# JokerJohn/Cloud_Map_Evaluation

Hardware: AMD Instinct MI355X
Metric: Mpts/sec full metric suite (CD+MME+AWD) on 50M-pt pair (higher is better)
Workload: dtype f64

## Files before the change

### cloud_map_evaluation_amd/csrc/me_internal.hpp

```cpp
#pragma once

#include <hip/hip_runtime.h>

#include <algorithm>
#include <cstdint>
#include <cstdlib>
#include <cstdio>
#include <map>
#include <string>
#include <vector>

#include "../../include/mapeval_hip.h"

namespace me {

constexpr int kFan = 8;
constexpr int kMaxLevels = 17;
constexpr int kMortonBits = 21;

struct DevBuf {
    void *p = nullptr;
    size_t bytes = 0;
    bool owned = true;
    ~DevBuf() { release(); }
// ... 773 lines not shown
    unsigned int lo = (unsigned int) __double2loint(v), hi = (unsigned int) __double2hiint(v);
    auto a = __builtin_amdgcn_permlane16_swap(lo, lo, false, false);
    auto b = __builtin_amdgcn_permlane16_swap(hi, hi, false, false);
    v = __hiloint2double((int) b[0], (int) a[0]) + __hiloint2double((int) b[1], (int) a[1]);
    lo = (unsigned int) __double2loint(v);
    hi = (unsigned int) __double2hiint(v);
    auto c = __builtin_amdgcn_permlane32_swap(lo, lo, false, false);
    auto d = __builtin_amdgcn_permlane32_swap(hi, hi, false, false);
    return __hiloint2double((int) d[0], (int) c[0]) + __hiloint2double((int) d[1], (int) c[1]);
}
template <int STAGE>
__device__ __forceinline__ int octet_partner_i(int v) {
    constexpr int ctrl = STAGE == 0 ? 0xB1 : (STAGE == 1 ? 0x4E : 0x141);
    return __builtin_amdgcn_update_dpp(0, v, ctrl, 0xF, 0xF, true);
}
template <int STAGE>
__device__ __forceinline__ double octet_partner_d(double v) {
    return __hiloint2double(octet_partner_i<STAGE>(__double2hiint(v)), octet_partner_i<STAGE>(__double2loint(v)));
}
template <int STAGE>
__device__ __forceinline__ long long octet_partner_ll(long long v) {
    const unsigned int lo = (unsigned int) octet_partner_i<STAGE>((int) (unsigned int) v);
    const unsigned int hi = (unsigned int) octet_partner_i<STAGE>((int) (unsigned int) ((unsigned long long) v >> 32));
    return (long long) (((unsigned long long) hi << 32) | lo);
}
__device__ __forceinline__ int wave_min_i(int v) {
    v = min(v, __builtin_amdgcn_update_dpp(0, v, 0xB1, 0xF, 0xF, true));
    v = min(v, __builtin_amdgcn_update_dpp(0, v, 0x4E, 0xF, 0xF, true));
    v = min(v, __builtin_amdgcn_update_dpp(0, v, 0x141, 0xF, 0xF, true));
    v = min(v, __builtin_amdgcn_update_dpp(0, v, 0x140, 0xF, 0xF, true));
    return min(min(__builtin_amdgcn_readlane(v, 0), __builtin_amdgcn_readlane(v, 16)),
               min(__builtin_amdgcn_readlane(v, 32), __builtin_amdgcn_readlane(v, 48)));
}
__device__ __forceinline__ int wave_max_i(int v) {
    v = max(v, __builtin_amdgcn_update_dpp(0, v, 0xB1, 0xF, 0xF, true));
    v = max(v, __builtin_amdgcn_update_dpp(0, v, 0x4E, 0xF, 0xF, true));
    v = max(v, __builtin_amdgcn_update_dpp(0, v, 0x141, 0xF, 0xF, true));
    v = max(v, __builtin_amdgcn_update_dpp(0, v, 0x140, 0xF, 0xF, true));
    return max(max(__builtin_amdgcn_readlane(v, 0), __builtin_amdgcn_readlane(v, 16)),
               max(__builtin_amdgcn_readlane(v, 32), __builtin_amdgcn_readlane(v, 48)));
}

constexpr int kGroupR = 2;
constexpr int kGroupTab = 343;
constexpr int kGroupTab2 = (2 * kGroupR + 5) * (2 * kGroupR + 5) * (2 * kGroupR + 5);

__host__ __device__ constexpr unsigned int recip14(int n) {
    return (unsigned int) (((n < 4 ? 0x1556200040000000ULL : 0x09250AAB0CCD1000ULL) >> (16 * (n & 3))) & 0xffffULL);
}
constexpr bool recip14_exact() {
    for (int n = 1; n <= 7; ++n)
        for (unsigned int t = 0; t < 5461; ++t)
            if (((t * recip14(n)) >> 14) != t / (unsigned int) n) return false;
    return true;
}
static_assert(recip14_exact(), "t / n as (t * recip14(n)) >> 14");
__host__ __device__ constexpr unsigned int spread11_32(unsigned int x) {
    x = (x | x << 16) & 0x070000ffu;
    x = (x | x << 8) & 0x0700f00fu;
    x = (x | x << 4) & 0x430c30c3u;
    x = (x | x << 2) & 0x49249249u;
    return x;
}
__host__ __device__ constexpr unsigned long long spread21_halves(unsigned int x) {
    return (unsigned long long) spread11_32(x & 0x3ffu) | ((unsigned long long) spread11_32((x >> 10) & 0x7ffu) << 30);
}
constexpr unsigned long long spread21_ladder(unsigned long long x) {
    x &= 0x1fffffULL;
    x = (x | x << 32) & 0x1f00000000ffffULL;
    x = (x | x << 16) & 0x1f0000ff0000ffULL;
    x = (x | x << 8) & 0x100f00f00f00f00fULL;
    x = (x | x << 4) & 0x10c30c30c30c30c3ULL;
    x = (x | x << 2) & 0x1249249249249249ULL;
    return x;
}
constexpr bool spread21_halves_exact() {
    for (unsigned int i = 0; i < 21; ++i) {
        const unsigned int a = 1u << i, b = (2u << i) - 1u, c = 0x1fffffu & ~(a - 1u);
        if (spread21_halves(a) != spread21_ladder(a) || spread21_halves(b) != spread21_ladder(b) || spread21_halves(c) != spread21_ladder(c)) return false;
    }
    for (unsigned int x = 0; x < 0x200000u; x += 4099u)
        if (spread21_halves(x) != spread21_ladder(x)) return false;
    return true;
}
static_assert(spread21_halves_exact(), "spread21 from 32-bit halves");
constexpr int kGroupRowsEnt = 240;
template <int H = 1, bool CULL = false, int R = kGroupR, bool MLP = false, bool ENT = false>
__device__ __forceinline__ bool wave_group_table(bool pending, int cx, int cy, int cz, const GridView &g, int cell_lim,
                                                 int lane, int2 *tab, GroupBox &box, int *n_keys_out = nullptr,
                                                 unsigned int *rows = nullptr, unsigned short *tcell = nullptr,
                                                 unsigned int *tabc = nullptr, const unsigned int *cell_aux = nullptr,
                                                 int *leader_out = nullptr) {
    const unsigned long long pm = __ballot(pending);
#ifdef ME_LEADER_FIRST
    const int leader = __ffsll((long long) pm) - 1;
#else
    const int rank = __popcll(pm & ((1ULL << lane) - 1ULL));
    const int n_pending = __popcll(pm);
    int leader = __ffsll((long long) __ballot(pending && rank == (n_pending >> 1))) - 1;
#ifndef ME_LEADER_MIDDLE
    {
        auto group_size = [&](int l) {
            const int ax = readlane_i(cx, l), ay = readlane_i(cy, l), az = readlane_i(cz, l);
            const int ux = cx - ax, uy = cy - ay, uz = cz - az;
            return __popcll(__ballot(pending && ux >= -R && ux <= R && uy >= -R && uy <= R && uz >= -R && uz <= R));
        };
        int best = group_size(leader);
        if (best < n_pending && n_pending >= 8) {
#pragma unroll
            for (int c = 1; c <= 5; ++c) {
                if (c == 3) continue;
                const int l = __ffsll((long long) __ballot(pending && rank == ((c * n_pending) / 6))) - 1;
                const int b = group_size(l);
                if (b > best) {
                    best = b;
                    leader = l;
                }
            }
        }
    }
#endif
#endif
    if (leader_out) *leader_out = leader;
    const int lx = readlane_i(cx, leader), ly = readlane_i(cy, leader), lz = readlane_i(cz, leader);
    const int ex = cx - lx, ey = cy - ly, ez = cz - lz;
    const bool in = pending && ex >= -R && ex <= R && ey >= -R && ey <= R && ez >= -R && ez <= R;
    const int x0 = __builtin_amdgcn_readfirstlane(wave_min_i(in ? cx : lx)) - H;
    const int x1 = __builtin_amdgcn_readfirstlane(wave_max_i(in ? cx : lx)) + H;
    const int y0 = __builtin_amdgcn_readfirstlane(wave_min_i(in ? cy : ly)) - H;
    const int y1 = __builtin_amdgcn_readfirstlane(wave_max_i(in ? cy : ly)) + H;
    const int z0 = __builtin_amdgcn_readfirstlane(wave_min_i(in ? cz : lz)) - H;
    const int z1 = __builtin_amdgcn_readfirstlane(wave_max_i(in ? cz : lz)) + H;
    const int nx = x1 - x0 + 1, ny = y1 - y0 + 1, nz = z1 - z0 + 1;
    const int n_keys = nx * ny * nz;
    if (n_keys_out) *n_keys_out = n_keys;
    box.x0 = x0;
    box.y0 = y0;
    box.z0 = z0;
    box.nx = nx;
    box.ny = ny;
    static_assert(!ENT || (H == 1 && R <= 2 && CULL && !MLP), "ENT: the <= 7 x 7 x 7 box of the stream kernels, with the cull");
    const unsigned int mx = ENT ? recip14(nx) : 0u, my = ENT ? recip14(ny) : 0u;
    unsigned long long *ykey = ENT ? reinterpret_cast<unsigned long long *>(rows + 128) : nullptr, *xkey = ENT ? ykey + 49 : nullptr;
    if (CULL) {
        const int n_rows = ny * nz;
        if (lane < n_rows) rows[lane] = 0u;
        __builtin_amdgcn_fence(__ATOMIC_ACQ_REL, "wavefront");
        __builtin_amdgcn_wave_barrier();
        if (in) atomicOr(&rows[(cy - y0) + ny * (cz - z0)], 1u << (cx - x0));
        __builtin_amdgcn_fence(__ATOMIC_ACQ_REL, "wavefront");
        __builtin_amdgcn_wave_barrier();
        if (lane < n_rows) {
            const int rz = ENT ? (int) (((unsigned int) lane * my) >> 14) : lane / ny, ry = lane - rz * ny;
            unsigned int m = 0;
            for (int dz = -H; dz <= H; ++dz)
                for (int dy = -H; dy <= H; ++dy) {
                    const int yy = ry + dy, zz = rz + dz;
                    if (yy >= 0 && yy < ny && zz >= 0 && zz < nz) m |= rows[yy + ny * zz];
                }
            unsigned int d = m;
#pragma unroll
            for (int s = 1; s <= H; ++s) d |= (m << s) | (m >> s);
            if (ENT) {
                const int iy = y0 + ry, iz = z0 + rz;
                const unsigned int okx = ((1u << (cell_lim - x0 < nx ? cell_lim - x0 : nx)) - 1u) & ~((1u << (x0 < 0 ? -x0 : 0)) - 1u);
                d = (iy >= 0 && iy < cell_lim && iz >= 0 && iz < cell_lim) ? d & okx : 0u;
                ykey[lane] = (spread21_halves((unsigned int) iy & 0x1fffffu) << 1) | (spread21_halves((unsigned int) iz & 0x1fffffu) << 2);
            }
            rows[64 + lane] = d;
        }
        if (ENT && lane < nx) xkey[lane] = spread21_halves((unsigned int) (x0 + lane) & 0x1fffffu);
        __builtin_amdgcn_fence(__ATOMIC_ACQ_REL, "wavefront");
        __builtin_amdgcn_wave_barrier();
    }
    if (MLP) {
        constexpr int NIT = ((2 * R + 1 + 2 * H) * (2 * R + 1 + 2 * H) * (2 * R + 1 + 2 * H) + 63) / 64;
        unsigned long long key[NIT], got[NIT];
        unsigned int slot[NIT];
        bool want[NIT];
#pragma unroll
        for (int i = 0; i < NIT; ++i) {
            const int t = lane + 64 * i;
            const int tx = t % nx, ty = (t / nx) % ny, tz = t / (nx * ny);
            const int ix = x0 + tx, iy = y0 + ty, iz = z0 + tz;
            want[i] = t < n_keys && ix >= 0 && iy >= 0 && iz >= 0 && ix < cell_lim && iy < cell_lim && iz < cell_lim;
            if (CULL) want[i] = want[i] && ((rows[64 + (t < n_keys ? ty + ny * tz : 0)] >> tx) & 1u);
            key[i] = spread21((unsigned long long) ix) | (spread21((unsigned long long) iy) << 1) | (spread21((unsigned long long) iz) << 2);
            slot[i] = (unsigned int) hash_u64(key[i]) & g.hmask;
            got[i] = kEmptyKey;
            if (tcell && t < n_keys) tcell[t] = (unsigned short) (tx | (ty << 3) | (tz << 6));
        }
#pragma unroll
        for (int i = 0; i < NIT; ++i)
            if (want[i]) got[i] = g.hkeys[slot[i]];
        int ci[NIT];
#pragma unroll
        for (int i = 0; i < NIT; ++i) {
            while (want[i] && got[i] != key[i] && got[i] != kEmptyKey) {
                slot[i] = (slot[i] + 1) & g.hmask;
                got[i] = g.hkeys[slot[i]];
            }
            want[i] = want[i] && got[i] == key[i];
            ci[i] = 0;
        }
#pragma unroll
        for (int i = 0; i < NIT; ++i)
            if (want[i]) ci[i] = (int) g.hvals[slot[i]];
        unsigned int cs0[NIT], cs1[NIT], ax[NIT];
#pragma unroll
        for (int i = 0; i < NIT; ++i) {
            cs0[i] = cs1[i] = ax[i] = 0;
            if (want[i]) {
                cs0[i] = g.cell_start[ci[i]];
                cs1[i] = g.cell_start[ci[i] + 1];
                if (tabc) ax[i] = cell_aux[ci[i]];
            }
        }
#pragma unroll
        for (int i = 0; i < NIT; ++i) {
            const int t = lane + 64 * i;
            if (t < n_keys) {
                tab[t] = make_int2((int) cs0[i], (int) (cs1[i] - cs0[i]));
                if (tabc) tabc[t] = ax[i];
            }
        }
    } else if (ENT) {
        for (int t = lane; t < n_keys; t += 64) {
            const unsigned int q = ((unsigned int) t * mx) >> 14, tx = (unsigned int) t - q * (unsigned int) nx;
            int2 run = make_int2(0, 0);
            if ((rows[64 + q] >> tx) & 1u) {
                const unsigned long long key = ykey[q] | xkey[tx];
                unsigned int s = (unsigned int) hash_u64(key) & g.hmask;
                for (;;) {
                    uint4 e = *reinterpret_cast<const uint4 *>(g.hent + s);
                    asm volatile("" : "+v"(e.x), "+v"(e.y), "+v"(e.z), "+v"(e.w));
                    const unsigned long long k = ((unsigned long long) e.y << 32) | e.x;
                    if (k == key) {
                        run = make_int2((int) e.z, (int) e.w);
                        break;
                    }
                    if (k == kEmptyKey) break;
                    s = (s + 1) & g.hmask;
                }
            }
            tab[t] = run;
            if (tcell) {
                const unsigned int tz = (q * my) >> 14, ty = q - tz * (unsigned int) ny;
                tcell[t] = (unsigned short) (tx | (ty << 3) | (tz << 6));
            }
        }
    } else
    for (int t = lane; t < n_keys; t += 64) {
        const int tx = t % nx, ty = (t / nx) % ny, tz = t / (nx * ny);
        const int ix = x0 + tx, iy = y0 + ty, iz = z0 + tz;
        int2 run = make_int2(0, 0);
        unsigned int aux = 0;
        bool want = ix >= 0 && iy >= 0 && iz >= 0 && ix < cell_lim && iy < cell_lim && iz < cell_lim;
        if (CULL) want = want && ((rows[64 + ty + ny * tz] >> tx) & 1u);
        if (want) {
            const unsigned long long key = spread21((unsigned long long) ix) | (spread21((unsigned long long) iy) << 1) |
                                           (spread21((unsigned long long) iz) << 2);
            const int ci = hash_lookup(g.hkeys, g.hvals, g.hmask, key);
            if (ci >= 0) {
                run.x = (int) g.cell_start[ci];
                run.y = (int) g.cell_start[ci + 1] - run.x;
                if (tabc) aux = cell_aux[ci];
            }
        }
        tab[t] = run;
        if (tabc) tabc[t] = aux;
        if (tcell) tcell[t] = (unsigned short) (tx | (ty << 3) | (tz << 6));
    }
    __builtin_amdgcn_fence(__ATOMIC_ACQ_REL, "wavefront");
    __builtin_amdgcn_wave_barrier();
    return in;
}
constexpr int kGroupRows = 128;

template <bool MERGE = false, class F>
__device__ __forceinline__ void wave_for_each_run(const int2 *tab, int n_keys, int lane, F &&f) {
    for (int base = 0; base < n_keys; base += 64) {
        const int t = base + lane;
        const int cnt = (t < n_keys) ? tab[t].y : 0;
        unsigned long long m = __ballot(cnt > 0);
        while (m) {
            const int n = __ffsll((long long) m) - 1;
            m &= m - 1;
            const int2 run = tab[base + n];
            const int cs = __builtin_amdgcn_readfirstlane(run.x);
            int cc = __builtin_amdgcn_readfirstlane(run.y);
            if (MERGE) {
                while (m) {
                    const int n2 = __ffsll((long long) m) - 1;
                    const int2 nx = tab[base + n2];
                    if (__builtin_amdgcn_readfirstlane(nx.x) != cs + cc) break;
                    cc += __builtin_amdgcn_readfirstlane(nx.y);
                    m &= m - 1;
                }
            }
            f(cs, cs + cc, base + n);
        }
    }
}
#endif

}
```

### cloud_map_evaluation_amd/csrc/me_mme.hip

```cpp
#include <cmath>
#include <cstdlib>

#include "me_internal.hpp"

#ifndef ME_MME_DEPTH
#define ME_MME_DEPTH 2
#endif
#ifndef ME_MME_DBG
#define ME_MME_DBG 0
#endif

namespace me {

__device__ __forceinline__ double half2_sum_d(double v) {
    unsigned int lo = (unsigned int) __double2loint(v), hi = (unsigned int) __double2hiint(v);
    auto c = __builtin_amdgcn_permlane32_swap(lo, lo, false, false);
    auto d = __builtin_amdgcn_permlane32_swap(hi, hi, false, false);
    return __hiloint2double((int) d[0], (int) c[0]) + __hiloint2double((int) d[1], (int) c[1]);
}


#ifdef ME_MME_STATS
__device__ unsigned long long g_mme_stat[8];
#endif

struct alignas(16) MmeTileRec {
    float4 f;
    double2 xy;
    double z;
    double pad;
};
static_assert(sizeof(MmeTileRec) == 48, "tile record layout");
template <class T>
__device__ __forceinline__ T lds_load(unsigned int addr) {
#if defined(__HIP_DEVICE_COMPILE__)
    return *reinterpret_cast<const __attribute__((address_space(3))) T *>((size_t) addr);
#else
    (void) addr;
    return T{};
#endif
}

template <int TILE, int WAVES>
__global__ void __launch_bounds__(256) __attribute__((amdgpu_waves_per_eu(WAVES, WAVES)))
k_mme3(const SPoint *__restrict__ sp, const unsigned long long *__restrict__ codes, long long i_begin, long long i_end,
       GridView g, FrameView fr, SlabView slab, double r2, int min_k, double *__restrict__ ent_s,
       unsigned char *__restrict__ valid_s, double *__restrict__ part_sum, long long *__restrict__ part_cnt,
       unsigned int xcd_chunk, int dbg, double cell_h, float thr_lo, float thr_hi, unsigned long long *__restrict__ part_pairs,
       unsigned int *__restrict__ refine_list, unsigned int *__restrict__ refine_count, double cond) {
    static_assert(TILE * sizeof(MmeTileRec) >= kGroupRowsEnt * 4, "the row masks and keys of the round's table alias the tile");
    (void) fr;
    (void) cell_h;
    const unsigned int vb = xcd_virtual_block(blockIdx.x, gridDim.x, xcd_chunk);
    const unsigned int loc = vb * blockDim.x + threadIdx.x;
    bool active = i_begin + (long long) loc < i_end;
    const int shift3 = 3 * g.shift;
    const int cell_lim = 1 << (kMortonBits - g.shift);

    unsigned long long mycell = ~0ULL;
    if (active) {
        const long long i = i_begin + (long long) loc;
        mycell = codes[i] >> shift3;
        if (slab.axis >= 0) {
            const SPoint q = sp[i];
            if (!slab_owned(slab, q.x, q.y, q.z)) {
                ent_s[i] = 0.0;
                valid_s[i] = 0;
                active = false;
            }
        }
    }
    bool done = !active;

    __shared__ int2 s_tab[4][kGroupTab + 1];
    __shared__ MmeTileRec s_rec[4][TILE];
    const int wv = __builtin_amdgcn_readfirstlane((int) (threadIdx.x >> 6));
    int2 *tab = s_tab[wv];
    MmeTileRec *trec = s_rec[wv];
    const unsigned int trec_lds = (unsigned int) (size_t) trec;
    const int lane = threadIdx.x & 63;

    unsigned int wave_pairs = 0;
    double det_keep = 0.0;
    bool have_det = false;
    bool thin = false;
#ifdef ME_MME_STATS
    int st_round = 0;
#endif
    while (__ballot(!done)) {
        GroupBox bx;
        int nk = 0, leader = 0;
        const int cx = (int) compact21(mycell), cy = (int) compact21(mycell >> 1), cz = (int) compact21(mycell >> 2);
        const bool in = wave_group_table<1, true, kGroupR, false, true>(!done, cx, cy, cz, g, cell_lim, lane, tab, bx, &nk, reinterpret_cast<unsigned int *>(trec),
                                                  nullptr, nullptr, nullptr, &leader);
        double qx = 0, qy = 0, qz = 0;
        if (!done) {
            unsigned int loc_q = loc;
            asm volatile("" : "+v"(loc_q));
            const SPoint q = sp[i_begin + (long long) loc_q];
            qx = q.x;
            qy = q.y;
            qz = q.z;
        }
        const double ox = uniform_f64(__hiloint2double(__builtin_amdgcn_readlane(__double2hiint(qx), leader), __builtin_amdgcn_readlane(__double2loint(qx), leader)));
        const double oy = uniform_f64(__hiloint2double(__builtin_amdgcn_readlane(__double2hiint(qy), leader), __builtin_amdgcn_readlane(__double2loint(qy), leader)));
        const double oz = uniform_f64(__hiloint2double(__builtin_amdgcn_readlane(__double2hiint(qz), leader), __builtin_amdgcn_readlane(__double2loint(qz), leader)));
        const double rx = qx - ox, ry = qy - oy, rz = qz - oz;
        const float ax = (float) (-2.0 * rx), ay = (float) (-2.0 * ry), az = (float) (-2.0 * rz);
        const float s = fmaf(az, az, fmaf(ay, ay, ax * ax));
        const float t_hi = (in && dbg != 2) ? fmaf(-0.25f, s, thr_hi) : -INFINITY;
        const float t_lo = (in && dbg != 2) ? fmaf(-0.25f, s, thr_lo) : -INFINITY;
        int k = -1;
        double s1x = -rx, s1y = -ry, s1z = -rz;
        double sxx = -(rx * rx), sxy = -(rx * ry), sxz = -(rx * rz), syy = -(ry * ry), syz = -(ry * rz), szz = -(rz * rz);
        if (!in || dbg == 2) {
            k = 0;
            s1x = s1y = s1z = sxx = sxy = sxz = syy = syz = szz = 0.0;
        }
#ifdef ME_MME_STATS
        int st_cand = 0;
#endif
        auto test = [&](const float4 &c, unsigned int ra, int gj) {
            const float u = fmaf(c.x, ax, fmaf(c.y, ay, fmaf(c.z, az, c.w)));
            const bool hi = u < t_hi;
            const unsigned long long mh = __ballot(hi);
            if (mh) {
                bool acc = u < t_lo;
                if (__builtin_expect(mh != __ballot(acc), 0)) {
                    asm volatile("; band: exact test" ::: "memory");
                    unsigned int loc_b = loc;
                    asm volatile("" : "+v"(loc_b));
                    const SPoint qe = sp[i_begin + (long long) loc_b];
                    const SPoint pe = sp[gj];
                    const double ex = pe.x - qe.x, ey = pe.y - qe.y, ez = pe.z - qe.z;
                    const double d2 = (ex * ex + ey * ey) + ez * ez;
                    acc = acc || (hi && d2 < r2);
                }
                if (acc) {
                    const double2 pxy = lds_load<double2>(ra + 16);
                    const double dx = pxy.x, dy = pxy.y, dz = lds_load<double>(ra + 32);
                    ++k;
                    s1x += dx;
                    s1y += dy;
                    s1z += dz;
                    sxx = fma(dx, dx, sxx);
                    sxy = fma(dx, dy, sxy);
                    sxz = fma(dx, dz, sxz);
                    syy = fma(dy, dy, syy);
                    syz = fma(dy, dz, syz);
                    szz = fma(dz, dz, szz);
                }
            }
        };
        if (dbg != 1) wave_for_each_run(tab, nk, lane, [&](int cs, int ce, int) {
            for (int base = cs; base < ce; base += TILE) {
                const int n = min(TILE, ce - base);
#ifdef ME_MME_STATS
                st_cand += n;
#endif
                if (lane < n) {
                    const SPoint p = sp[base + lane];
                    const double px = p.x - ox, py = p.y - oy, pz = p.z - oz;
                    const float fx = (float) px, fy = (float) py, fz = (float) pz;
                    const double w = ((double) fx * (double) fx + (double) fy * (double) fy) + (double) fz * (double) fz;
                    trec[lane].f = make_float4(fx, fy, fz, (float) w);
                    trec[lane].xy = make_double2(px, py);
                    trec[lane].z = pz;
                }
                __builtin_amdgcn_fence(__ATOMIC_ACQ_REL, "wavefront");
                __builtin_amdgcn_wave_barrier();
                int j = (dbg == 3) ? n : 0;
                unsigned int ra = trec_lds;
                asm volatile("" : "+v"(ra));
                for (; j + 2 <= n; j += 2) {
                    const float4 c0 = lds_load<float4>(ra), c1 = lds_load<float4>(ra + (unsigned int) sizeof(MmeTileRec));
                    test(c0, ra, base + j);
                    test(c1, ra + (unsigned int) sizeof(MmeTileRec), base + j + 1);
                    ra += 2u * (unsigned int) sizeof(MmeTileRec);
                    asm volatile("" : "+v"(ra));
                }
                for (; j < n; ++j) {
                    const float4 c0 = lds_load<float4>(ra);
                    test(c0, ra, base + j);
                    ra += (unsigned int) sizeof(MmeTileRec);
                    asm volatile("" : "+v"(ra));
                }
                __builtin_amdgcn_fence(__ATOMIC_ACQ_REL, "wavefront");
                __builtin_amdgcn_wave_barrier();
            }
        });
#ifdef ME_MME_STATS
        {
            int ka = in ? k : 0;
            for (int o = 32; o > 0; o >>= 1) ka += __shfl_xor(ka, o, 64);
            const int served = __popcll(__ballot(in));
            if (lane == 0) {
                atomicAdd(&g_mme_stat[0], 1ULL);
                atomicAdd(&g_mme_stat[1], (unsigned long long) st_cand);
                atomicAdd(&g_mme_stat[2], (unsigned long long) served);
                atomicAdd(&g_mme_stat[3], (unsigned long long) ka);
                if (st_round > 0) {
                    atomicAdd(&g_mme_stat[4], 1ULL);
                    atomicAdd(&g_mme_stat[5], (unsigned long long) st_cand);
                    atomicAdd(&g_mme_stat[6], (unsigned long long) served);
                }
            }
            ++st_round;
        }
#endif
        if (part_pairs) {
            int ka = in ? k : 0;
            for (int o = 32; o > 0; o >>= 1) ka += __shfl_xor(ka, o, 64);
            wave_pairs += (unsigned int) __builtin_amdgcn_readfirstlane(ka);
        }
        if (in) {
            done = true;
            const int kk = k;
            if (kk >= min_k) {
                const double inv_k = 1.0 / (double) kk, inv_km1 = 1.0 / (double) (kk - 1);
                const double cxx = (sxx - s1x * s1x * inv_k) * inv_km1;
                const double cxy = (sxy - s1x * s1y * inv_k) * inv_km1;
                const double cxz = (sxz - s1x * s1z * inv_k) * inv_km1;
                const double cyy = (syy - s1y * s1y * inv_k) * inv_km1;
                const double cyz = (syz - s1y * s1z * inv_k) * inv_km1;
                const double czz = (szz - s1z * s1z * inv_k) * inv_km1;
                det_keep = cxx * (cyy * czz - cyz * cyz) - cxy * (cxy * czz - cyz * cxz) + cxz * (cxy * cyz - cyy * cxz);
                have_det = true;
                const double tr = (cxx + cyy) + czz;
                thin = det_keep < 0.25 * tr * tr * cond;
            }
        }
        __builtin_amdgcn_wave_barrier();
    }
    if (refine_list) {
        const unsigned long long tm = __ballot(thin);
        if (tm) {
            unsigned int base = 0;
            if (lane == 0) base = atomicAdd(refine_count, (unsigned int) __popcll(tm));
            base = (unsigned int) readlane_i((int) base, 0);
            if (thin) refine_list[base + (unsigned int) __popcll(tm & ((1ULL << lane) - 1ULL))] = loc;
        }
    }
    double H = 0.0;
    bool ok = false;
    if (active) {
        if (have_det) {
            const double h = 0.5 * log(2.0 * M_PI * M_E * det_keep);
            if (!isnan(h) && !isinf(h)) {
                H = h;
                ok = true;
            }
        }
        unsigned int loc_e = loc;
        asm volatile("" : "+v"(loc_e));
        const long long i = i_begin + (long long) loc_e;
        ent_s[i] = H;
        valid_s[i] = ok ? 1 : 0;
    }
    __shared__ double smd[4];
    __shared__ long long smi[4];
    const double bs = block_sum_256(H, smd);
    const long long bc = block_sum_256_ll(ok ? 1LL : 0LL, smi);
    if (threadIdx.x == 0) {
        part_sum[blockIdx.x] = bs;
        part_cnt[blockIdx.x] = bc;
    }
    if (part_pairs) {
        __shared__ unsigned int smp[4];
        if (lane == 0) smp[wv] = wave_pairs;
        __syncthreads();
        if (threadIdx.x == 0) part_pairs[blockIdx.x] = (unsigned long long) smp[0] + smp[1] + smp[2] + smp[3];
    }
}


constexpr int kRefineBlock = 256;
__global__ void __launch_bounds__(kRefineBlock)
k_mme_refine(const SPoint *__restrict__ sp, const unsigned long long *__restrict__ codes, long long i_begin, GridView g, double r2,
             int min_k, const unsigned int *__restrict__ list, unsigned int n_list, double *__restrict__ ent_s,
             unsigned char *__restrict__ valid_s) {
    __shared__ int2 s_runs[kRefineBlock / 8][28];
    const int sub = threadIdx.x & 7, oct = threadIdx.x >> 3;
    const unsigned int t = blockIdx.x * (kRefineBlock / 8) + oct;
    const bool alive = t < n_list;
    const long long i = i_begin + (long long) (alive ? list[t] : 0u);
    const SPoint q = sp[alive ? i : i_begin];
    const unsigned long long cell = codes[alive ? i : i_begin] >> (3 * g.shift);
    const int cx = (int) compact21(cell), cy = (int) compact21(cell >> 1), cz = (int) compact21(cell >> 2);
    const int cell_lim = 1 << (kMortonBits - g.shift);
    {
        unsigned long long key[4], got[4];
        unsigned int slot[4];
        bool want[4];
#pragma unroll
        for (int u = 0; u < 4; ++u) {
            const int c = sub + 8 * u;
            const int ix = cx + (c % 3) - 1, iy = cy + ((c / 3) % 3) - 1, iz = cz + (c / 9) - 1;
            want[u] = alive && c < 27 && ix >= 0 && iy >= 0 && iz >= 0 && ix < cell_lim && iy < cell_lim && iz < cell_lim;
            key[u] = spread21((unsigned long long) ix) | (spread21((unsigned long long) iy) << 1) | (spread21((unsigned long long) iz) << 2);
            slot[u] = (unsigned int) hash_u64(key[u]) & g.hmask;
            got[u] = kEmptyKey;
        }
#pragma unroll
        for (int u = 0; u < 4; ++u)
            if (want[u]) got[u] = g.hkeys[slot[u]];
        unsigned int ci[4], c0[4], c1[4];
#pragma unroll
        for (int u = 0; u < 4; ++u) {
            while (want[u] && got[u] != key[u] && got[u] != kEmptyKey) {
                slot[u] = (slot[u] + 1) & g.hmask;
                got[u] = g.hkeys[slot[u]];
            }
            want[u] = want[u] && got[u] == key[u];
            ci[u] = 0;
        }
#pragma unroll
        for (int u = 0; u < 4; ++u)
            if (want[u]) ci[u] = g.hvals[slot[u]];
#pragma unroll
        for (int u = 0; u < 4; ++u) {
            c0[u] = c1[u] = 0;
            if (want[u]) {
                c0[u] = g.cell_start[ci[u]];
                c1[u] = g.cell_start[ci[u] + 1];
            }
        }
#pragma unroll
        for (int u = 0; u < 4; ++u)
            if (sub + 8 * u < 27) s_runs[oct][sub + 8 * u] = make_int2((int) c0[u], (int) (c1[u] - c0[u]));
    }
    __builtin_amdgcn_fence(__ATOMIC_ACQ_REL, "wavefront");
    __builtin_amdgcn_wave_barrier();
    auto scan = [&](auto &&f) {
        for (int c = 0; c < 27; ++c) {
            const int2 run = s_runs[oct][c];
            for (int j0 = 0; j0 < run.y; j0 += 32) {
                SPoint p[4];
#pragma unroll
                for (int u = 0; u < 4; ++u) p[u] = sp[run.x + min(j0 + sub + 8 * u, run.y - 1)];
#pragma unroll
                for (int u = 0; u < 4; ++u) {
                    const double dx = p[u].x - q.x, dy = p[u].y - q.y, dz = p[u].z - q.z;
                    const double d2 = (dx * dx + dy * dy) + dz * dz;
                    if (j0 + sub + 8 * u < run.y && d2 < r2) f(dx, dy, dz);
                }
            }
        }
    };
    auto oct_sum = [](double v) {
        v += octet_partner_d<0>(v);
        v += octet_partner_d<1>(v);
        v += octet_partner_d<2>(v);
        return v;
    };
    int cnt = 0;
    double s1x = 0, s1y = 0, s1z = 0;
    scan([&](double dx, double dy, double dz) {
        ++cnt;
        s1x += dx;
        s1y += dy;
        s1z += dz;
    });
    cnt += octet_partner_i<0>(cnt);
    cnt += octet_partner_i<1>(cnt);
    cnt += octet_partner_i<2>(cnt);
    s1x = oct_sum(s1x);
    s1y = oct_sum(s1y);
    s1z = oct_sum(s1z);
    const int kk = cnt - 1;
    double H = 0.0;
    bool ok = false;
    if (kk >= min_k) {
        const double mx = s1x / (double) kk, my = s1y / (double) kk, mz = s1z / (double) kk;
        double sxx = 0, sxy = 0, sxz = 0, syy = 0, syz = 0, szz = 0;
        scan([&](double dx, double dy, double dz) {
            const double ex = dx - mx, ey = dy - my, ez = dz - mz;
            sxx = fma(ex, ex, sxx);
            sxy = fma(ex, ey, sxy);
            sxz = fma(ex, ez, sxz);
            syy = fma(ey, ey, syy);
            syz = fma(ey, ez, syz);
            szz = fma(ez, ez, szz);
        });
        sxx = oct_sum(sxx);
        sxy = oct_sum(sxy);
        sxz = oct_sum(sxz);
        syy = oct_sum(syy);
        syz = oct_sum(syz);
        szz = oct_sum(szz);
        sxx -= mx * mx;
        sxy -= mx * my;
        sxz -= mx * mz;
        syy -= my * my;
        syz -= my * mz;
        szz -= mz * mz;
        const double inv = 1.0 / (double) (kk - 1);
        const double cxx = sxx * inv, cxy = sxy * inv, cxz = sxz * inv, cyy = syy * inv, cyz = syz * inv, czz = szz * inv;
        const double det = cxx * (cyy * czz - cyz * cyz) - cxy * (cxy * czz - cyz * cxz) + cxz * (cxy * cyz - cyy * cxz);
        const double h = 0.5 * log(2.0 * M_PI * M_E * det);
        if (!isnan(h) && !isinf(h)) {
            H = h;
            ok = true;
        }
    }
    if (alive && sub == 0) {
        ent_s[i] = H;
        valid_s[i] = ok ? 1 : 0;
    }
}

__global__ void __launch_bounds__(256)
k_mme_resum(const double *__restrict__ ent_s, const unsigned char *__restrict__ valid_s, long long i_begin, long long i_end,
            double *__restrict__ part_sum, long long *__restrict__ part_cnt) {
    const long long i = i_begin + (long long) blockIdx.x * 256 + threadIdx.x;
    double H = 0.0;
    long long ok = 0;
    if (i < i_end) {
        H = ent_s[i];
        ok = valid_s[i] ? 1 : 0;
    }
    __shared__ double smd[4];
    __shared__ long long smi[4];
    const double bs = block_sum_256(H, smd);
    const long long bc = block_sum_256_ll(ok, smi);
    if (threadIdx.x == 0) {
        part_sum[blockIdx.x] = bs;
        part_cnt[blockIdx.x] = bc;
    }
}

__global__ void __launch_bounds__(256) k_sum_u64(const unsigned long long *__restrict__ v, long long n, unsigned long long *__restrict__ out) {
    long long s = 0;
    for (long long i = threadIdx.x; i < n; i += 256) s += (long long) v[i];
    __shared__ long long sm[4];
    const long long r = block_sum_256_ll(s, sm);
    if (threadIdx.x == 0) *out += (unsigned long long) r;
}

#ifdef ME_AB
#include "me_mme_kernels_ab.inc"
#endif

__global__ void k_mme_unpermute(const SPoint *__restrict__ sp, long long i_begin, long long i_end,
                                const double *__restrict__ ent_s, const unsigned char *__restrict__ valid_s,
                                double *__restrict__ ent_o, unsigned char *__restrict__ valid_o) {
    const long long i = i_begin + (long long) blockIdx.x * blockDim.x + threadIdx.x;
    if (i >= i_end) return;
    const long long o = sp[i].idx;
    if (ent_o) ent_o[o] = ent_s[i];
    if (valid_o) valid_o[o] = valid_s[i];
}

__global__ void __launch_bounds__(256)
k_mme_final(const double *__restrict__ ps, const long long *__restrict__ pc, long long nb, long long chunk,
            double *__restrict__ out_s, long long *__restrict__ out_c) {
    double s = 0;
    long long c = 0;
    const long long b0 = (long long) blockIdx.x * chunk, b1 = b0 + chunk < nb ? b0 + chunk : nb;
    for (long long b = b0 + threadIdx.x; b < b1; b += 256) {
        s += ps[b];
        c += pc[b];
    }
    __shared__ double smd[4];
    __shared__ long long smi[4];
    const double rs = block_sum_256(s, smd);
    const long long rc = block_sum_256_ll(c, smi);
    if (threadIdx.x == 0) {
        out_s[blockIdx.x] = rs;
        out_c[blockIdx.x] = rc;
    }
}

static int mme_unpermute_to_host(me_ctx *ctx, Cloud &c, long long b, long long e, double *entropies, uint8_t *valid) {
    const long long n = c.n;
    DevBuf &eo = ctx->tmp[2], &vo = ctx->tmp[3];
    ME_CHECK(ctx, eo.ensure((size_t) n * 8));
    ME_CHECK(ctx, vo.ensure((size_t) n));
    if (ctx->shard_world > 1) {
        ME_CHECK(ctx, hipMemsetAsync(eo.p, 0, (size_t) n * 8, ctx->stream));
        ME_CHECK(ctx, hipMemsetAsync(vo.p, 0, (size_t) n, ctx->stream));
    }
    if (e > b)
        hipLaunchKernelGGL(k_mme_unpermute, dim3((unsigned int) ((e - b + 255) / 256)), dim3(256), 0, ctx->stream, c.sp.as<SPoint>(), b, e,
                           c.mme_ent.as<double>(), c.mme_val.as<unsigned char>(), entropies ? eo.as<double>() : nullptr,
                           valid ? vo.as<unsigned char>() : nullptr);
    if (entropies) ME_TRY(copy_d2h(ctx, entropies, eo.p, (size_t) n * 8));
    if (valid) ME_TRY(copy_d2h(ctx, valid, vo.p, (size_t) n));
    return ME_OK;
}

__global__ void k_mme_repermute(const SPoint *__restrict__ sp, long long n, const double *__restrict__ ent_o,
                                const unsigned char *__restrict__ valid_o, double *__restrict__ ent_s, unsigned char *__restrict__ valid_s) {
    const long long i = (long long) blockIdx.x * blockDim.x + threadIdx.x;
    if (i >= n) return;
    const long long o = sp[i].idx;
    ent_s[i] = ent_o[o];
    valid_s[i] = valid_o[o];
}

int mme_carry_out(me_ctx *ctx, int slot) {
    Cloud &c = ctx->cloud[slot];
    if (!c.mme_have || c.n == 0) return ME_OK;
    ME_CHECK(ctx, ctx->mme_keep_e.ensure((size_t) c.n * 8));
    ME_CHECK(ctx, ctx->mme_keep_v.ensure((size_t) c.n));
    hipLaunchKernelGGL(k_mme_unpermute, dim3((unsigned int) ((c.n + 255) / 256)), dim3(256), 0, ctx->stream, c.sp.as<SPoint>(), 0LL, c.n,
                       c.mme_ent.as<double>(), c.mme_val.as<unsigned char>(), ctx->mme_keep_e.as<double>(),
                       ctx->mme_keep_v.as<unsigned char>());
    ctx->mme_keep_n = c.n;
    return ME_OK;
}

int mme_carry_in(me_ctx *ctx, int slot) {
    Cloud &c = ctx->cloud[slot];
    if (ctx->mme_keep_n != c.n || c.n == 0 || !c.index_valid) return ME_OK;
    ME_CHECK(ctx, c.mme_ent.ensure((size_t) c.n * 8));
    ME_CHECK(ctx, c.mme_val.ensure((size_t) c.n));
    hipLaunchKernelGGL(k_mme_repermute, dim3((unsigned int) ((c.n + 255) / 256)), dim3(256), 0, ctx->stream, c.sp.as<SPoint>(), c.n,
                       ctx->mme_keep_e.as<double>(), ctx->mme_keep_v.as<unsigned char>(), c.mme_ent.as<double>(),
                       c.mme_val.as<unsigned char>());
    c.mme_have = true;
    ctx->mme_keep_n = -1;
    return ME_OK;
}

int mme_fetch(me_ctx *ctx, int slot, double *entropies, uint8_t *valid) {
    if (slot < 0 || slot > 1) return ctx->fail(ME_ERR_ARG, "bad slot");
    Cloud &c = ctx->cloud[slot];
    if (!c.uploaded || !c.mme_have) return ctx->fail(ME_ERR_STATE, "me_mme_fetch: no MME result for this slot (run me_mme or me_run_suite first)");
    if (c.n == 0 || (!entropies && !valid)) return ME_OK;
    ME_CHECK(ctx, hipSetDevice(ctx->device));
    long long b, e;
    ctx->shard_range(c.n, b, e);
    ME_TRY(mme_unpermute_to_host(ctx, c, b, e, entropies, valid));
    ME_CHECK(ctx, hipStreamSynchronize(ctx->stream));
    return ME_OK;
}

int mme_run(me_ctx *ctx, int slot, double radius, int min_k, double *entropies, uint8_t *valid, double *sum_H,
            long long *n_valid) {
    if (slot < 0 || slot > 1) return ctx->fail(ME_ERR_ARG, "bad slot");
    if (!(radius > 0)) return ctx->fail(ME_ERR_ARG, "me_mme: radius must be > 0");
    if (min_k < 2) return ctx->fail(ME_ERR_ARG, "me_mme: min_k must be >= 2 (covariance divides by k-1)");
    Cloud &c = ctx->cloud[slot];
    if (!c.uploaded) return ctx->fail(ME_ERR_STATE, "me_mme: cloud not uploaded");
    if (c.slab.axis >= 0 && c.slab.reg_lo > -INFINITY && c.slab.lo - c.slab.reg_lo < radius)
        return ctx->fail(ME_ERR_ARG, "me_mme: slab halo is smaller than the radius");
    if (c.n == 0) {
        if (sum_H) *sum_H = 0.0;
        if (n_valid) *n_valid = 0;
        return ME_OK;
    }
    ME_TRACE_POINT(ctx, "mme_run: enter");
    ME_CHECK(ctx, hipSetDevice(ctx->device));
    const double want_h = radius * (1.0 + 0x1p-20);
    if (!c.index_valid || c.cell_h < want_h || c.cell_h > 1.5 * want_h) ME_TRY(cloud_build_index(ctx, slot, radius));
    const long long n = c.n;
    long long b, e;
    ctx->shard_range(n, b, e);
#ifdef ME_AB
#include "me_mme_prepare_ab.inc"
#endif
    DevBuf &ent_s = c.mme_ent, &val_s = c.mme_val;
    c.mme_have = false;
    ME_CHECK(ctx, ent_s.ensure((size_t) n * 8));
    ME_CHECK(ctx, val_s.ensure((size_t) n));
    const unsigned int nb = (unsigned int) std::max<long long>(8, ((e - b + 255) / 256 + 7) / 8 * 8);
    constexpr int kStage = 256;
    ME_TRACE_POINT(ctx, "mme_run: buffers ensured");
    ME_CHECK(ctx, ctx->red.ensure((size_t) (nb + kStage + 1) * 16 + 64));
    double *ps = ctx->red.as<double>();
    long long *pc = reinterpret_cast<long long *>(ps + nb);
    double *ps2 = reinterpret_cast<double *>(pc + nb);
    long long *pc2 = reinterpret_cast<long long *>(ps2 + kStage);
    double *outs = reinterpret_cast<double *>(pc2 + kStage);
    long long *outc = reinterpret_cast<long long *>(outs + 1);
    const double r2 = radius * radius;
    {
        const FrameView fr{c.origin[0], c.origin[1], c.origin[2], c.fine_h};
        const float band = (float) (0x1p-12 * c.cell_h * c.cell_h);
        const float thr_lo = (float) r2 - band, thr_hi = (float) r2 + band;
        unsigned long long *d_pairs = nullptr;
#ifndef ME_NO_PAIR_COUNT
        if (ctx->timers_on) {
            ME_CHECK(ctx, ctx->mme_pairs_buf.ensure((size_t) (nb + 2) * 8));
            d_pairs = ctx->mme_pairs_buf.as<unsigned long long>() + 2;
        }
#endif
        ME_CHECK(ctx, ctx->mme_refine.ensure((size_t) (e - b + 1) * 4 + 64));
        unsigned int *d_refine = ctx->mme_refine.as<unsigned int>();
        ME_CHECK(ctx, hipMemsetAsync(d_refine, 0, 4, ctx->stream));
        const double cond = ME_TUNE_MME_REFINE_COND * c.cell_h * c.cell_h;
        TimerScope ts(ctx, "mme");
#define ME_LAUNCH_MME3(T, W, DBG)                                                                                             \
    hipLaunchKernelGGL((k_mme3<T, W>), dim3(nb), dim3(256), 0, ctx->stream, c.sp.as<SPoint>(),                                \
                       c.codes.as<unsigned long long>(), b, e, c.grid, fr, c.slab, r2, min_k, ent_s.as<double>(),             \
                       val_s.as<unsigned char>(), ps, pc, xcd_chunk_setting(), DBG, c.cell_h, thr_lo, thr_hi, d_pairs, d_refine + 1,      \
                       d_refine, cond)
#ifdef ME_AB
#include "me_mme_dispatch_ab.inc"
#else
        ME_LAUNCH_MME3(32, ME_TUNE_MME_WAVES, ME_MME_DBG);
#endif
#undef ME_LAUNCH_MME3
        ts.end();
        ME_TRACE_POINT(ctx, "mme_run: k_mme3 queued");
        if (d_pairs) {
            unsigned long long *tot = ctx->mme_pairs_buf.as<unsigned long long>();
            ME_CHECK(ctx, hipMemsetAsync(tot, 0, 8, ctx->stream));
            hipLaunchKernelGGL(k_sum_u64, dim3(1), dim3(256), 0, ctx->stream, d_pairs, (long long) nb, tot);
            unsigned long long h = 0;
            {
                MailGuard mg(ctx);
                ME_TRY(mail_post(ctx, &h, tot, 8));
                ME_TRY(mg.sync());
            }
            ctx->mme_pairs += (long long) h;
        }
    }
    ME_TRACE_POINT(ctx, "mme_run: kernel launched");
    const long long chunk = ((long long) nb + kStage - 1) / kStage;
    hipLaunchKernelGGL(k_mme_final, dim3(kStage), dim3(256), 0, ctx->stream, ps, pc, (long long) nb, chunk, ps2, pc2);
    hipLaunchKernelGGL(k_mme_final, dim3(1), dim3(256), 0, ctx->stream, ps2, pc2, (long long) kStage, (long long) kStage, outs, outc);
    double hs = 0;
    long long hc = 0;
    unsigned int n_thin = 0;
    {
        MailGuard mg(ctx);
        ME_TRY(mail_post(ctx, &hs, outs, 8));
        ME_TRY(mail_post(ctx, &hc, outc, 8));
        ME_TRY(mail_post(ctx, &n_thin, ctx->mme_refine.as<unsigned int>(), 4));
        ME_TRY(mg.sync());
    }
    if (n_thin > 0) {
        ME_TRACE_POINT(ctx, "mme_run: refining thin neighbourhoods");
        {
            TimerScope ts(ctx, "mme_refine");
            hipLaunchKernelGGL(k_mme_refine, dim3((n_thin + kRefineBlock / 8 - 1) / (kRefineBlock / 8)), dim3(kRefineBlock), 0, ctx->stream,
                               c.sp.as<SPoint>(), c.codes.as<unsigned long long>(), b, c.grid, r2, min_k,
                               (const unsigned int *) (ctx->mme_refine.as<unsigned int>() + 1), n_thin, ent_s.as<double>(), val_s.as<unsigned char>());
        }
        const unsigned int nb2 = (unsigned int) ((e - b + 255) / 256);
        hipLaunchKernelGGL(k_mme_resum, dim3(nb2), dim3(256), 0, ctx->stream, (const double *) ent_s.as<double>(),
                           (const unsigned char *) val_s.as<unsigned char>(), b, e, ps, pc);
        const long long chunk2 = ((long long) nb2 + kStage - 1) / kStage;
        hipLaunchKernelGGL(k_mme_final, dim3(kStage), dim3(256), 0, ctx->stream, ps, pc, (long long) nb2, chunk2, ps2, pc2);
        hipLaunchKernelGGL(k_mme_final, dim3(1), dim3(256), 0, ctx->stream, ps2, pc2, (long long) kStage, (long long) kStage, outs, outc);
        MailGuard mg(ctx);
        ME_TRY(mail_post(ctx, &hs, outs, 8));
        ME_TRY(mail_post(ctx, &hc, outc, 8));
        ME_TRY(mg.sync());
        ctx->mme_refined += (long long) n_thin;
    }
    if (entropies || valid) ME_TRY(mme_unpermute_to_host(ctx, c, b, e, entropies, valid));
    ME_TRACE_POINT(ctx, "mme_run: synced");
    ME_CHECK(ctx, hipGetLastError());
#ifdef ME_MME_STATS
    {
        unsigned long long st[8] = {0}, zero[8] = {0};
        (void) hipMemcpyFromSymbol(st, HIP_SYMBOL(g_mme_stat), sizeof st);
        (void) hipMemcpyToSymbol(HIP_SYMBOL(g_mme_stat), zero, sizeof zero);
        if (st[0])
            std::fprintf(stderr, "[mme stats] queries=%lld pass rounds=%llu (%.3f per 16 queries) candidates/round=%.1f queries served/round=%.1f accepted/query=%.1f | MFMA blocks/round=%.2f steps taken/round=%.2f (of %.2f) pairs/step=%.1f\n",
                         (long long) (e - b), st[0], (double) st[0] * 16.0 / (double) (e - b), (double) st[1] / (double) st[0],
                         (double) st[2] / (double) st[0], (double) st[3] / (double) (e - b) - 1.0, (double) st[4] / (double) st[0],
                         (double) st[5] / (double) st[0], 4.0 * (double) st[4] / (double) st[0],
                         st[5] ? (double) st[3] / (double) st[5] : 0.0);
    }
#endif
    c.mme_have = true;
    if (sum_H) *sum_H = hs;
    if (n_valid) *n_valid = hc;
    return ME_OK;
}

}
```

Baseline: 2363.

## Pack candidate runs into full tiles across run boundaries in MME kernel

Instead of staging each contiguous candidate run separately (leaving partial tiles per run), the kernel compacts the run table into a prefix-summed list and stages fixed-size tiles spanning multiple runs. It uses a head bitmask and mbcnt to map each lane to its run. The global index is stored in the tile record for the exact-test path. The tile size is raised from 32 to 48. This cuts underfilled tile iterations, at the cost of extra scan, bitmask and LDS work per tile.

After: 2451, median of 6. +3.7%, better.

```diff
diff --git a/cloud_map_evaluation_amd/csrc/me_internal.hpp b/cloud_map_evaluation_amd/csrc/me_internal.hpp
--- a/cloud_map_evaluation_amd/csrc/me_internal.hpp
+++ b/cloud_map_evaluation_amd/csrc/me_internal.hpp
@@ -1099,6 +1099,39 @@
         }
     }
 }
-#endif
-
-}
+
+__device__ __forceinline__ int wave_incl_scan_i(int v, int lane, int *total) {
+    v += __builtin_amdgcn_update_dpp(0, v, 0x111, 0xF, 0xF, true);
+    v += __builtin_amdgcn_update_dpp(0, v, 0x112, 0xF, 0xF, true);
+    v += __builtin_amdgcn_update_dpp(0, v, 0x114, 0xF, 0xF, true);
+    v += __builtin_amdgcn_update_dpp(0, v, 0x118, 0xF, 0xF, true);
+    const int t0 = __builtin_amdgcn_readlane(v, 15), t1 = t0 + __builtin_amdgcn_readlane(v, 31), t2 = t1 + __builtin_amdgcn_readlane(v, 47);
+    *total = t2 + __builtin_amdgcn_readlane(v, 63);
+    return v + (lane < 32 ? (lane < 16 ? 0 : t0) : (lane < 48 ? t1 : t2));
+}
+
+__device__ __forceinline__ int wave_run_list(int2 *tab, int n_keys, int lane, int *n_runs) {
+    int nr = 0, total = 0;
+    for (int base = 0; base < n_keys; base += 64) {
+        const int t = base + lane;
+        int2 run = make_int2(0, 0);
+        if (t < n_keys) run = tab[t];
+        const unsigned long long m = __ballot(run.y > 0);
+        int batch = 0;
+        const int incl = wave_incl_scan_i(run.y, lane, &batch);
+        const int rank = (int) __builtin_amdgcn_mbcnt_hi((unsigned int) (m >> 32), __builtin_amdgcn_mbcnt_lo((unsigned int) m, 0u));
+        __builtin_amdgcn_fence(__ATOMIC_ACQ_REL, "wavefront");
+        __builtin_amdgcn_wave_barrier();
+        if (run.y > 0) tab[nr + rank] = make_int2(run.x, total + incl - run.y);
+        nr += __popcll(m);
+        total += batch;
+    }
+    if (lane == 0) tab[nr] = make_int2(0, total);
+    __builtin_amdgcn_fence(__ATOMIC_ACQ_REL, "wavefront");
+    __builtin_amdgcn_wave_barrier();
+    *n_runs = nr;
+    return total;
+}
+#endif
+
+}
diff --git a/cloud_map_evaluation_amd/csrc/me_mme.hip b/cloud_map_evaluation_amd/csrc/me_mme.hip
--- a/cloud_map_evaluation_amd/csrc/me_mme.hip
+++ b/cloud_map_evaluation_amd/csrc/me_mme.hip
@@ -28,7 +28,8 @@
     float4 f;
     double2 xy;
     double z;
-    double pad;
+    int gi;
+    int pad;
 };
 static_assert(sizeof(MmeTileRec) == 48, "tile record layout");
 template <class T>
@@ -77,6 +78,8 @@
     const int wv = __builtin_amdgcn_readfirstlane((int) (threadIdx.x >> 6));
     int2 *tab = s_tab[wv];
     MmeTileRec *trec = s_rec[wv];
+    __shared__ unsigned int s_head[4][2];
+    unsigned int *head = s_head[wv];
     const unsigned int trec_lds = (unsigned int) (size_t) trec;
     const int lane = threadIdx.x & 63;
 
@@ -120,7 +123,7 @@
 #ifdef ME_MME_STATS
         int st_cand = 0;
 #endif
-        auto test = [&](const float4 &c, unsigned int ra, int gj) {
+        auto test = [&](const float4 &c, unsigned int ra) {
             const float u = fmaf(c.x, ax, fmaf(c.y, ay, fmaf(c.z, az, c.w)));
             const bool hi = u < t_hi;
             const unsigned long long mh = __ballot(hi);
@@ -131,7 +134,7 @@
                     unsigned int loc_b = loc;
                     asm volatile("" : "+v"(loc_b));
                     const SPoint qe = sp[i_begin + (long long) loc_b];
-                    const SPoint pe = sp[gj];
+                    const SPoint pe = sp[lds_load<int>(ra + 40)];
                     const double ex = pe.x - qe.x, ey = pe.y - qe.y, ez = pe.z - qe.z;
                     const double d2 = (ex * ex + ey * ey) + ez * ez;
                     acc = acc || (hi && d2 < r2);
@@ -152,21 +155,40 @@
                 }
             }
         };
-        if (dbg != 1) wave_for_each_run(tab, nk, lane, [&](int cs, int ce, int) {
-            for (int base = cs; base < ce; base += TILE) {
-                const int n = min(TILE, ce - base);
+        static_assert(TILE <= 64, "a chunk is staged by one wave, its head mask is two words");
+        if (dbg != 1) {
+            int n_runs = 0;
+            const int total = wave_run_list(tab, nk, lane, &n_runs);
+            int s_r0 = 0;
+            for (int base = 0; base < total; base += TILE) {
+                const int n = min(TILE, total - base);
 #ifdef ME_MME_STATS
                 st_cand += n;
 #endif
+                if (lane < 2) head[lane] = 0u;
+                __builtin_amdgcn_fence(__ATOMIC_ACQ_REL, "wavefront");
+                __builtin_amdgcn_wave_barrier();
+                if (s_r0 + 1 + lane < n_runs) {
+                    const int d = tab[s_r0 + 1 + lane].y - base - 1;
+                    if (d < TILE) atomicOr(&head[d >> 5], 1u << (d & 31));
+                }
+                __builtin_amdgcn_fence(__ATOMIC_ACQ_REL, "wavefront");
+                __builtin_amdgcn_wave_barrier();
+                const unsigned int h0 = (unsigned int) __builtin_amdgcn_readfirstlane((int) head[0]);
+                const unsigned int h1 = (unsigned int) __builtin_amdgcn_readfirstlane((int) head[1]);
                 if (lane < n) {
-                    const SPoint p = sp[base + lane];
+                    const int2 run = tab[s_r0 + (int) __builtin_amdgcn_mbcnt_hi(h1, __builtin_amdgcn_mbcnt_lo(h0, 0u))];
+                    const int gi = run.x + (base + lane - run.y);
+                    const SPoint p = sp[gi];
                     const double px = p.x - ox, py = p.y - oy, pz = p.z - oz;
                     const float fx = (float) px, fy = (float) py, fz = (float) pz;
                     const double w = ((double) fx * (double) fx + (double) fy * (double) fy) + (double) fz * (double) fz;
                     trec[lane].f = make_float4(fx, fy, fz, (float) w);
                     trec[lane].xy = make_double2(px, py);
                     trec[lane].z = pz;
-                }
+                    trec[lane].gi = gi;
+                }
+                s_r0 += __popc(h0) + __popc(h1);
                 __builtin_amdgcn_fence(__ATOMIC_ACQ_REL, "wavefront");
                 __builtin_amdgcn_wave_barrier();
                 int j = (dbg == 3) ? n : 0;
@@ -174,21 +196,21 @@
                 asm volatile("" : "+v"(ra));
                 for (; j + 2 <= n; j += 2) {
                     const float4 c0 = lds_load<float4>(ra), c1 = lds_load<float4>(ra + (unsigned int) sizeof(MmeTileRec));
-                    test(c0, ra, base + j);
-                    test(c1, ra + (unsigned int) sizeof(MmeTileRec), base + j + 1);
+                    test(c0, ra);
+                    test(c1, ra + (unsigned int) sizeof(MmeTileRec));
                     ra += 2u * (unsigned int) sizeof(MmeTileRec);
                     asm volatile("" : "+v"(ra));
                 }
                 for (; j < n; ++j) {
                     const float4 c0 = lds_load<float4>(ra);
-                    test(c0, ra, base + j);
+                    test(c0, ra);
                     ra += (unsigned int) sizeof(MmeTileRec);
                     asm volatile("" : "+v"(ra));
                 }
                 __builtin_amdgcn_fence(__ATOMIC_ACQ_REL, "wavefront");
                 __builtin_amdgcn_wave_barrier();
             }
-        });
+        }
 #ifdef ME_MME_STATS
         {
             int ka = in ? k : 0;
@@ -599,7 +621,7 @@
 #ifdef ME_AB
 #include "me_mme_dispatch_ab.inc"
 #else
-        ME_LAUNCH_MME3(32, ME_TUNE_MME_WAVES, ME_MME_DBG);
+        ME_LAUNCH_MME3(48, ME_TUNE_MME_WAVES, ME_MME_DBG);
 #endif
 #undef ME_LAUNCH_MME3
         ts.end();
```
